# pedrosecchi67/ImmersedBoundary.jl

Hardware: AMD Instinct MI355X
Metric: Mcells*iters/s residual sweep (advection-JST-MUSCL), 2D RAE2822 (higher is better)
Workload: dtype f32

## Files before the change

### immersedboundary.jl_amd/csrc/ibh_common.h

```cpp
#pragma once
#include <hip/hip_runtime.h>
#include <stdint.h>
#include <string>
#include <vector>

#include "../../include/ibhip.h"

#define IBH_MAXD 3

enum : int32_t { SIDE_SAME = 0, SIDE_MIRROR = 1, SIDE_COARSE = 2, SIDE_FINE = 3, SIDE_GENERAL = 4 };

struct BlockDesc2 {
    int32_t base;
    int32_t type[4];
    int32_t nb[4][2];
    int32_t sub[4];
    float h[2];
    float rh[2];
    float q[4];
    float rt[4];
    int32_t dt;
};

struct QuadDesc2 {
    int32_t base;
    uint32_t cls;
    float rh[2];
};
#define IBH_QROW 160
#define IBH_QAUX 40
struct QuadSet2 {
    std::vector<QuadDesc2> qd;
    std::vector<int32_t> qtab;
    std::vector<int32_t> qaux, paux;
    std::vector<int32_t> singles;
    int32_t nq_int = 0, ns_int = 0;
    std::vector<QuadDesc2> pd;
    std::vector<int32_t> ptab;
    std::vector<int32_t> singles2;
};

struct BlockDesc3 {
    int32_t base;
    int32_t fine;
    int32_t type[6];
    int32_t nb[6];
    int32_t sub[6];
    float h[3];
    float rh[3];
    float q[6];
    float rt[6];
};

struct DimData {
    int32_t nf = 0;
    int32_t *owners = nullptr, *neighbors = nullptr;
    int32_t *loff = nullptr, *lidx = nullptr;
    int32_t *roff = nullptr, *ridx = nullptr;
};

struct ibh_part {
    int nd = 0;
    int32_t nc = 0;
    float* spacing = nullptr;
    float* centers = nullptr;
    DimData dim[IBH_MAXD];
    int32_t* side = nullptr;
    int32_t n_image = 0;
    int32_t* image_in_domain = nullptr;
    int bs = 0;
    int32_t nblk = 0;
    int32_t nA1 = 0, nB1 = 0;
    BlockDesc2* blocks2 = nullptr;
    int32_t* htab = nullptr;
    int32_t* etab = nullptr;
    int32_t* dtab = nullptr;
    int32_t n_dt = 0;
    int32_t* img_list = nullptr;
    int32_t n_img = 0, n_img_int = 0, img_all_fz = 0;
    int32_t fuse_all = 0;
    int32_t rows_ok = 0;
    QuadDesc2* qd[2] = {nullptr, nullptr};
    int32_t* qtab[2] = {nullptr, nullptr};
    int32_t* qaux[2] = {nullptr, nullptr};
    int32_t* qsingles[2] = {nullptr, nullptr};
    int32_t nq[2] = {0, 0}, nq_int[2] = {0, 0}, nqs[2] = {0, 0}, nqs_int[2] = {0, 0};
    int32_t npair = 0, nqs2 = 0;
    int32_t* qsingles2 = nullptr;
    int32_t* fz_list = nullptr;
    int32_t* ng_list = nullptr;
    int32_t* nf_list = nullptr;
    int32_t n_fz = 0, n_fz_int = 0, n_ng = 0, n_ng_int = 0, n_nf = 0, n_nf_int = 0;
    BlockDesc3* blocks3 = nullptr;
    int32_t* htab3 = nullptr;
    int32_t* ftab3 = nullptr;
    int32_t *rtab3 = nullptr, *r4tab3 = nullptr;
    int32_t sweep3 = 0;
    BlockDesc3* iblocks3 = nullptr;
    int32_t *ihtab3 = nullptr, *iftab3 = nullptr, *irtab3 = nullptr, *ir4tab3 = nullptr, *idtab3 = nullptr;
    int32_t n_img3 = 0, img_all3 = 0;
    int32_t n_irr = 0;
    int32_t* irr_cells = nullptr;
    int32_t* irr_rec = nullptr;
    int64_t info[24] = {0};
    float* G = nullptr;
    float* march_tmp = nullptr;
    size_t march_tmp_n = 0;
    size_t G_bytes = 0;
};

struct ibh_acc {
    int32_t n_out = 0, n_in = 0;
    int32_t *off = nullptr, *idx = nullptr;
    float* w = nullptr;
    float* packed = nullptr;
};

struct ibh_bc {
    int32_t ng = 0, nid = 0;
    int32_t *ghost = nullptr, *image_domain = nullptr;
    float* eta = nullptr;
    ibh_acc interp;
    std::vector<int32_t> h_ghost, h_off, h_donor;
    std::vector<float> h_eta, h_w;
};

#define IBH_MAX_BC 8
struct ibh_bcset {
    int nbc = 0, nlev = 0;
    int32_t ng = 0;
    int32_t seg[IBH_MAX_BC + 1] = {0};
    bool direct[IBH_MAX_BC] = {false};
    unsigned int* sync = nullptr;
    int32_t *ghost = nullptr, *off = nullptr, *donor = nullptr, *bidx = nullptr;
    float *eta = nullptr, *w = nullptr, *gval = nullptr, *value = nullptr;
    int32_t* mode = nullptr;
};

extern "C" int ibh_shear_rate_of_velocity_cells(const ibh_part* p, const float* vel, int64_t ldv, float* S, float* Gout,
                                                int64_t ldg);
extern "C" int ibh_wray_agarwal_of_cells(const ibh_part* p, const float* R, const float* S, float sigmaR, float C1,
                                         float kappa, float* nut, float* nuR, float* Sout);

extern "C" int ibh_scalar_transport_blocks(const ibh_part* p, const float* R, const float* nuR, float nu, const float* vel,
                                           int64_t ldv, const float* S, float* out, int* done);

extern "C" int ibh_bcset_apply_with_dt(const ibh_bcset* s, float* a, ibh_part* p, const float* C, int64_t ldc, float scale,
                                       float* dt_next, int partials_done);

extern "C" {
extern int ibh_viscous_per_cell;
extern int ibh_ew_scalar_only;
extern int ibh_time_average_nt;
}

extern thread_local std::string ibh_err;
extern thread_local hipStream_t ibh_stream;

int ibh_fail(int code, const char* what, const char* file, int line);

#define IBH_HIP(call)                                                        \
// ... 72 lines not shown
```

### immersedboundary.jl_amd/csrc/ibh_fused.hip

```cpp
#include <algorithm>

#include <string.h>

#include "ibh_common.h"
#include "ibh_flux.h"

using namespace ibhf;

namespace {

struct PartView {
    int32_t nc;
    const float* spacing;
    DimData dim[IBH_MAXD];
    const int32_t* side;
};

struct SideIter {
    int32_t b, e, o, n;
    const int32_t* idx;
    bool direct;
};
__device__ __forceinline__ SideIter side_iter(const PartView& p, int d, int side, int32_t c) {
    const DimData& dd = p.dim[d];
    SideIter it;
    it.idx = side ? dd.ridx : dd.lidx;
    const int32_t t = p.side[(int64_t)(2 * d + side) * p.nc + c];
    it.direct = t >= 0;
    it.o = side ? c : t;
    it.n = side ? t : c;
    if (t >= 0) {
        it.b = 0;
        it.e = 1;
    } else if (t == -2) {
        it.b = it.e = 0;
    } else {
        const int32_t* off = side ? dd.roff : dd.loff;
        it.b = off[c];
        it.e = off[c + 1];
    }
    return it;
}
__device__ __forceinline__ void side_face(const DimData& dd, const SideIter& it, int32_t k, int32_t& o, int32_t& n) {
    if (it.direct) {
        o = it.o;
        n = it.n;
    } else {
        const int32_t f = it.idx[k];
        o = dd.owners[f];
        n = dd.neighbors[f];
    }
}

template <int ND, int NV>
// ... 1125 lines not shown
            F = F * 1.0f;
        }
        Hf[s * 64 + lane] = F;
    }
    blk2::wave_lds_sync();
    const int i = lane & 7, j = lane >> 3;
    const bool e0 = i == 0, e1 = i == 7, e2 = j == 0, e3 = j == 7;
    const float fzl = Hf[4 * 64 + lane], fzh = Hf[5 * 64 + lane];
#pragma unroll
    for (int k = 0; k < 8; ++k) {
        const uint32_t c = base + lane + 64 * k;
        const float *r = tR + k * 64, *t = tT + k * 64, *ax = tAx + k * 64, *ay = tAy + k * 64;
        const float Rc = Rk[k], Tc = Tk[k];
        float fl[3], fr[3];
        const int xl = e0 ? lane : lane - 1, xr = e1 ? lane : lane + 1, yl = e2 ? lane : lane - 8, yr = e3 ? lane : lane + 8;
        const float fxl = tr3_flux(r[xl], Rc, t[xl], Tc, ax[xl], Ak[0][k], h[0], h[0]) * 1.0f;
        const float fxr = tr3_flux(Rc, r[xr], Tc, t[xr], Ak[0][k], ax[xr], h[0], h[0]) * 1.0f;
        const float fyl = tr3_flux(r[yl], Rc, t[yl], Tc, ay[yl], Ak[1][k], h[1], h[1]) * 1.0f;
        const float fyr = tr3_flux(Rc, r[yr], Tc, t[yr], Ak[1][k], ay[yr], h[1], h[1]) * 1.0f;
        fl[0] = e0 ? Hf[0 * 64 + j + 8 * k] : fxl;
        fr[0] = e1 ? Hf[1 * 64 + j + 8 * k] : fxr;
        fl[1] = e2 ? Hf[2 * 64 + i + 8 * k] : fyl;
        fr[1] = e3 ? Hf[3 * 64 + i + 8 * k] : fyr;
        const int kl = k > 0 ? k - 1 : 0, kh = k < 7 ? k + 1 : 7;
        const float fzl_in = tr3_flux(Rk[kl], Rc, Tk[kl], Tc, Ak[2][kl], Ak[2][k], h[2], h[2]) * 1.0f;
        const float fzr_in = tr3_flux(Rc, Rk[kh], Tc, Tk[kh], Ak[2][k], Ak[2][kh], h[2], h[2]) * 1.0f;
        fl[2] = k == 0 ? fzl : fzl_in;
        fr[2] = k == 7 ? fzh : fzr_in;
        float rt = ldg(S, c);
#pragma unroll
        for (int d = 0; d < 3; ++d) rt = rt + (fr[d] - fl[d]) / h[d];
        out[c] = rt;
    }
}


int env_int(const char* name, int dflt) {
    const char* s = getenv(name);
    return s ? atoi(s) : dflt;
}
struct Tuning {
    int wave3d = env_int("IBH_3D_WAVE", 1);
    int sweep_iters = env_int("IBH_SWEEP_ITERS", 0);
    int quad = env_int("IBH_QUAD", 1);
    int rows = env_int("IBH_ROWS", 0);
    int quad_variant = env_int("IBH_QUAD_VARIANT", 0);
    int quad_parts = 3, quad_singles_iters = 1;
    int quad_singles_first = env_int("IBH_SINGLES_FIRST", 0);
    int pairs = env_int("IBH_PAIRS", 1);
    int arith_ids = env_int("IBH_ARITH_IDS", 1);
    int transport_blocks = 1;
    int rows_singles = env_int("IBH_ROWS_SINGLES", -1);
} T;
#define IBH_ROWS_SINGLES_MIN 24000

enum : int {
    QV_STAMPS = 4,
    QV_GATHER_5 = 5, QV_GATHER_69 = 69, QV_GATHER_85 = 85, QV_GATHER_NONE = 100,
    QV_GATHER_SEVEN = 126,
    QV_THREAD_PER_CELL = 512,
    QV_STRIP_W2 = 515, QV_STRIP_W4 = 514, QV_STRIP_W3 = 518,
    QV_COLS_W4 = 519, QV_COLS_W5 = 520,
    QV_EULER_PERSISTENT = 514,
};

constexpr int F_LITERAL = IBH_FORCE_GENERAL | IBH_EXACT;
constexpr int F_TWO_KERNEL = IBH_NO_FUSE | IBH_PASS_A_ONLY | IBH_PASS_B_ONLY;
constexpr int F_PHASES = IBH_PHASE_INTERIOR | IBH_PHASE_BOUNDARY;

bool has_blocks(const ibh_part* p) { return p->bs == 8 && p->nblk > 0 && (p->nd == 2 ? !!p->blocks2 : !!p->blocks3); }
bool tuned2(const ibh_part* p, int flags) { return p->nd == 2 && has_blocks(p) && !(flags & F_LITERAL); }
bool tuned3(const ibh_part* p, int flags) { return p->nd == 3 && has_blocks(p) && !(flags & F_LITERAL); }
bool fused2(const ibh_part* p, int flags) { return tuned2(p, flags) && !(flags & F_TWO_KERNEL); }
bool whole3(const ibh_part* p, int flags) { return tuned3(p, flags) && !(flags & (F_TWO_KERNEL | F_PHASES)); }
bool image3(const ibh_part* p, int flags) { return whole3(p, flags) && (flags & IBH_IMAGE_ONLY) && p->img_all3; }
bool single3(const ibh_part* p, int flags) { return whole3(p, flags) && !(flags & IBH_IMAGE_ONLY) && p->sweep3; }
bool all_blocks3(const ibh_part* p) {
    return p->nd == 3 && has_blocks(p) && p->n_irr == 0 && (int64_t)p->nblk * 512 == p->nc && p->info[6] == 0;
}
bool quads_usable(const ibh_part* p, int k, int flags) { return T.quad && !(flags & IBH_NO_QUAD) && p->nq[k] > 0; }

struct Range { int32_t first, last; int32_t count() const { return last - first; } };
struct Phase {
    bool interior, boundary;
    explicit Phase(int flags) : interior((flags & IBH_PHASE_INTERIOR) != 0), boundary((flags & IBH_PHASE_BOUNDARY) != 0) {}
    bool any() const { return interior || boundary; }
    bool valid() const { return !(interior && boundary); }
    Range of(int32_t n_int, int32_t n_all) const { return {boundary ? n_int : 0, interior ? n_int : n_all}; }
};
#define IBH_PHASES_EXCLUSIVE "IBH_PHASE_INTERIOR and IBH_PHASE_BOUNDARY are exclusive"

PartView view(const ibh_part* p) { return {p->nc, p->spacing, {p->dim[0], p->dim[1], p->dim[2]}, p->side}; }
FlatRec flat_of(const ibh_part* p, const int32_t* cells) {
    return cells && cells == p->irr_cells && p->irr_rec ? FlatRec{p->irr_rec, p->n_irr} : FlatRec{nullptr, 0};
}

int ensure_G(ibh_part* p) {
    if (p->G) return 0;
    hipStreamCaptureStatus st = hipStreamCaptureStatusNone;
    if (ibh_stream && hipStreamIsCapturing(ibh_stream, &st) == hipSuccess && st != hipStreamCaptureStatusNone)
        return ibh_fail(-1, "the gradient workspace is allocated on the first two-kernel sweep of a partition: run one "
                            "sweep before capturing it into a HIP graph", __FILE__, __LINE__);
    const size_t bytes = (size_t)(p->nd * (p->nd + 2) + 1) * (size_t)p->nc * sizeof(float);
    IBH_HIP(hipMalloc((void**)&p->G, bytes));
    p->G_bytes = bytes;
    return 0;
}

struct AdvArgs { const float *u, *C; int64_t ldc; float* ud; };
struct EulerArgs { const float* P; int64_t ldp; float* R; int64_t ldr; const ibh_fluid* fluid; };

struct QuadRange { Range q, s; };
QuadRange quad_range(const ibh_part* p, int k, Phase ph) {
    QuadRange r{ph.of(p->nq_int[k], p->nq[k]), ph.of(p->nqs_int[k], p->nqs[k])};
    if (T.quad_parts == 1) r.s.last = r.s.first;
    if (T.quad_parts == 2) r.q.last = r.q.first;
    return r;
}

struct BlockList { const BlockDesc2* bl; const int32_t *ht, *et, *ls; int32_t count, iters, nwg; };
BlockList block_list(const ibh_part* p, const int32_t* list, Range r, int wpb, int max_iters) {
    const int32_t count = r.count(), iters = T.sweep_iters > 0 ? T.sweep_iters : std::min(max_iters, std::max(1, count / 6000));
    return {list ? p->blocks2 : p->blocks2 + r.first, list ? p->htab : p->htab + (size_t)r.first * 64,
            list ? p->etab : p->etab + (size_t)r.first * 16, list ? list + r.first : nullptr, count, iters,
            (count + wpb * iters - 1) / (wpb * iters)};
}

struct Blocks3 { Range a, b; int32_t nI, gI; bool doA, doB; PartView v; FlatRec flat; };
Blocks3 blocks3_setup(const ibh_part* p, int flags, Phase ph) {
    const Range a = ph.of(p->nA1, p->nblk), b = ph.of(p->nB1, p->nblk);
    const int32_t nI = ph.interior ? 0 : p->n_irr, gI = (nI + 511) / 512;
    return {a, b, nI, gI, !(flags & IBH_PASS_B_ONLY) && (a.count() > 0 || gI), !(flags & IBH_PASS_A_ONLY) && (b.count() > 0 || gI),
            view(p), flat_of(p, p->irr_cells)};
}

struct CellLists { const int32_t *cellsA, *cellsB; int32_t nA, nB; };
CellLists cell_lists(const ibh_part* p, int flags, bool fast, Phase ph) {
    const bool image = (flags & IBH_IMAGE_ONLY) && !fast;
    const int32_t* cellsA = fast ? p->irr_cells : nullptr;
    const int32_t nA = fast ? (ph.interior ? 0 : p->n_irr) : p->nc;
    return {cellsA, image ? p->image_in_domain : cellsA, nA, image ? p->n_image : nA};
}
}

enum AdvPath {
    ADV3_IMAGE_COLS,
    ADV3_SINGLE,
    ADV3_BLOCKS,
    ADV2_IMAGE,
    ADV2_FUSE_ALL,
    ADV2_MIXED,
    ADV_GENERAL_2D,
    ADV_GENERAL_2D_EXACT,
    ADV_GENERAL_3D,
};
static AdvPath advection_path(const ibh_part* p, int flags) {
    if (tuned3(p, flags)) return image3(p, flags) ? ADV3_IMAGE_COLS : single3(p, flags) ? ADV3_SINGLE : ADV3_BLOCKS;
    if (fused2(p, flags)) {
        if ((flags & IBH_IMAGE_ONLY) && p->img_all_fz && !p->fuse_all) return ADV2_IMAGE;
        if (p->fuse_all) return ADV2_FUSE_ALL;
        const bool mixed_pays = p->n_fz >= 12000 || (flags & (IBH_FORCE_MIXED | IBH_SWEEP_ONLY));
        if (p->fz_list && 4 * (int64_t)p->n_fz >= p->nblk && mixed_pays) return ADV2_MIXED;
    }
    return p->nd != 2 ? ADV_GENERAL_3D : (flags & IBH_EXACT) ? ADV_GENERAL_2D_EXACT : ADV_GENERAL_2D;
}

static void adv3_image_cols(const ibh_part* p, const AdvArgs& a) {
    const int32_t nwg = (p->n_img3 + WPB3C - 1) / WPB3C;
    hipLaunchKernelGGL((k_sweep3_cols<3, true>), dim3(nwg), dim3(64 * WPB3C), 0, ibh_stream, a.u, a.C, (uint32_t)a.ldc, a.ud,
                       p->iblocks3, p->ihtab3, p->iftab3, p->irtab3, p->ir4tab3, p->n_img3, nwg, p->idtab3);
}
#define SWEEP3_LAUNCH(K)                                                                                                 \
    hipLaunchKernelGGL(K, dim3(nwg), dim3(64 * WPB3S), 0, ibh_stream, a.u, a.C, (uint32_t)a.ldc, a.ud, p->blocks3, p->htab3, \
                       p->ftab3, p->rtab3, p->r4tab3, p->nblk, nwg)
static void adv3_single(const ibh_part* p, const AdvArgs& a) {
    static_assert(WPB3C == WPB3S, "one grid for both forms");
    const int32_t nwg = (p->nblk + WPB3S - 1) / WPB3S;
    switch (T.quad_variant) {
    case QV_THREAD_PER_CELL:
        hipLaunchKernelGGL(k_sweep3_adv, dim3(p->nblk), dim3(512), 0, ibh_stream, a.u, a.C, (uint32_t)a.ldc, a.ud, p->blocks3,
                           p->htab3, p->ftab3, p->rtab3, p->r4tab3, p->nblk);
        break;
    case QV_STRIP_W2: SWEEP3_LAUNCH(k_sweep3_strip<2>); break;
    case QV_STRIP_W4: SWEEP3_LAUNCH(k_sweep3_strip<4>); break;
    case QV_STRIP_W3: SWEEP3_LAUNCH(k_sweep3_strip<3>); break;
    case QV_COLS_W4: SWEEP3_LAUNCH(k_sweep3_cols<4>); break;
    case QV_COLS_W5: SWEEP3_LAUNCH(k_sweep3_cols<5>); break;
    default: SWEEP3_LAUNCH(k_sweep3_cols<3>);
    }
}
#undef SWEEP3_LAUNCH

static int adv3_blocks(ibh_part* p, const AdvArgs& a, int flags, Phase ph) {
    if (const int rc = ensure_G(p)) return rc;
    const Blocks3 s = blocks3_setup(p, flags, ph);
    const int32_t na = s.a.count(), nb = s.b.count();
    if (s.doA && T.wave3d) {
        const int32_t nwgA = (na + 3) / 4, gIw = (s.nI + 255) / 256;
        hipLaunchKernelGGL(k_passA3_wave, dim3(nwgA + gIw), dim3(256), 0, ibh_stream, s.v, a.u, p->G, p->blocks3 + s.a.first,
                           p->htab3 + (size_t)s.a.first * 384, p->ftab3, na, nwgA, p->irr_cells, s.nI, s.flat,
                           (const int32_t*)nullptr);
    } else if (s.doA)
        hipLaunchKernelGGL(k_passA3_blk, dim3(na + s.gI), dim3(512), 0, ibh_stream, s.v, a.u, p->G, p->blocks3 + s.a.first,
                           p->htab3 + (size_t)s.a.first * 384, p->ftab3, na, p->irr_cells, s.nI, s.flat);
    if (s.doB)
        hipLaunchKernelGGL(k_passB3_adv_blk, dim3(nb + s.gI), dim3(512), 0, ibh_stream, s.v, a.u, a.C, a.ldc, p->G, a.ud,
                           p->blocks3 + s.b.first, p->htab3 + (size_t)s.b.first * 384, p->ftab3, nb, p->irr_cells, s.nI,
                           s.flat, (const int32_t*)nullptr);
    return 0;
}

static void adv2_block_list(const ibh_part* p, const AdvArgs& a, const int32_t* list, Range r) {
    if (r.count() <= 0) return;
    const BlockList L = block_list(p, list, r, WPB, 6);
    hipLaunchKernelGGL(p->n_dt > 0 ? k_sweep_adv<true> : k_sweep_adv<false>, dim3(L.nwg), dim3(64 * WPB), 0, ibh_stream, a.u,
                       a.C, (uint32_t)a.ldc, a.ud, L.bl, L.ht, L.et, p->dtab, L.count, L.nwg, L.iters, L.ls);
}

static void adv2_quads(const ibh_part* p, const AdvArgs& a, int k, Phase ph) {
    const Range q = quad_range(p, k, ph).q;
    Range s = quad_range(p, k, ph).s;
    const int32_t npair = (k == 0 && T.pairs && p->npair > 0 && !ph.boundary && q.first == 0 && q.last == p->nq[k] &&
                           T.quad_parts == 3) ? p->npair : 0;
    const int32_t* slist = p->qsingles[k];
    if (npair) {
        slist = p->qsingles2;
        s = {0, p->nqs2};
    } else if (k == 0 && p->npair > 0 && ph.boundary) {
        s.last = s.first;
    }
    const bool rows_able = k == 0 && p->rows_ok && p->n_dt == 0 && T.quad_variant == 0 && s.count() > 0;
    const bool rows_inside = rows_able && T.rows_singles == 2;
    const bool rows_second = rows_able && !rows_inside &&
                             (T.rows_singles < 0 ? s.count() >= IBH_ROWS_SINGLES_MIN : T.rows_singles > 0);
    const Range rs = s;
    if (rows_second) s.last = s.first;
    const int32_t siters = T.quad_singles_iters > 0 ? T.quad_singles_iters : 1;
    const int32_t nwgq = (q.count() + npair + WPB - 1) / WPB,
                  nwgs = rows_inside ? (s.count() + WPB * 8 - 1) / (WPB * 8) : (s.count() + WPB * siters - 1) / (WPB * siters);
    auto kq = k_sweep_quad<false, false>;
    if (rows_inside) kq = k_sweep_quad<false, false, 127, false, true>;
    else if (p->n_dt > 0) kq = k_sweep_quad<true, false>;
    else if (T.quad_variant == QV_STAMPS) kq = k_sweep_quad<false, true>;
    else if (T.quad_variant == QV_GATHER_SEVEN) kq = k_sweep_quad<false, false, 126>;
    else if (T.quad_variant == QV_GATHER_85) kq = k_sweep_quad<false, false, 85>;
    else if (T.quad_variant == QV_GATHER_69) kq = k_sweep_quad<false, false, 69>;
    else if (T.quad_variant == QV_GATHER_5) kq = k_sweep_quad<false, false, 5>;
    else if (T.quad_variant == QV_GATHER_NONE) kq = k_sweep_quad<false, false, 0>;
    if (nwgq + nwgs > 0)
        hipLaunchKernelGGL(kq, dim3(nwgq + nwgs), dim3(64 * WPB), 0, ibh_stream, a.u, a.C, (uint32_t)a.ldc, a.ud,
                           p->qd[k] + q.first, p->qtab[k] + (size_t)q.first * IBH_QROW, q.count(), nwgq, p->blocks2, p->htab,
                           p->etab, p->dtab, slist + s.first, s.count(), nwgs, T.quad_singles_first, siters,
                           (const float*)nullptr, npair,
                           T.arith_ids ? p->qaux[k] + (size_t)q.first * IBH_QAUX : (const int32_t*)nullptr);
    if (rows_second) {
        const int32_t nw = (rs.count() + 7) / 8, nwgr = (nw + WPBR - 1) / WPBR;
        hipLaunchKernelGGL(k_sweep_rows, dim3(nwgr), dim3(64 * WPBR), 0, ibh_stream, a.u, a.C, (uint32_t)a.ldc, a.ud,
                           p->blocks2, p->etab, 0, rs.count(), nwgr, slist + rs.first);
    }
}

static void adv2_single(const ibh_part* p, const AdvArgs& a, int flags, Phase ph, int k) {
    const Range b = k ? ph.of(p->n_img_int, p->n_img) : ph.of(p->nB1, p->nblk);
    if (k == 0 && p->rows_ok && T.rows && !(flags & IBH_NO_QUAD) && T.quad_variant == 0) {
        const int32_t nw = (b.count() + 7) / 8, nwg = (nw + WPBR - 1) / WPBR;
        if (nwg > 0)
            hipLaunchKernelGGL(k_sweep_rows, dim3(nwg), dim3(64 * WPBR), 0, ibh_stream, a.u, a.C, (uint32_t)a.ldc, a.ud,
                               p->blocks2, p->etab, b.first, b.count(), nwg, (const int32_t*)nullptr);
    } else if (quads_usable(p, k, flags)) adv2_quads(p, a, k, ph);
    else adv2_block_list(p, a, k ? p->img_list : nullptr, b);
}

static int adv2_mixed(ibh_part* p, const AdvArgs& a, int flags, Phase ph) {
    const bool defer = p->n_nf_int == 0;
    const Range g = ph.of(defer ? 0 : p->n_ng_int, p->n_ng), r = ph.of(p->n_nf_int, p->n_nf);
    const int32_t nI = ph.interior ? 0 : p->n_irr, gI = (nI + 64 * WPB - 1) / (64 * WPB);
    if (const int rc = ensure_G(p)) return rc;
    const int32_t nwgA = (g.count() + WPB - 1) / WPB, nwgB = (r.count() + WPB - 1) / WPB;
    if (!(flags & IBH_SWEEP_ONLY)) {
        const PartView v = view(p);
        if (nwgA + gI)
            hipLaunchKernelGGL((k_passA<2, 1, false>), dim3(nwgA + gI), dim3(64 * WPB), 0, ibh_stream, v, a.u, (int64_t)p->nc,
                               p->G, p->blocks2, p->htab, g.count(), nwgA, p->irr_cells, nI, flat_of(p, p->irr_cells),
                               p->ng_list + g.first);
        if (nwgB + gI)
            hipLaunchKernelGGL((k_passB_adv<2, false>), dim3(nwgB + gI), dim3(64 * WPB), 0, ibh_stream, v, a.u, a.C, a.ldc,
                               p->G, a.ud, p->blocks2, p->htab, r.count(), nwgB, p->irr_cells, nI,
                               flat_of(p, p->irr_cells), p->nf_list + r.first);
    }
    adv2_block_list(p, a, p->fz_list, ph.of(p->n_fz_int, p->n_fz));
    return 0;
}

static int adv_general(ibh_part* p, const AdvArgs& a, int flags, Phase ph, AdvPath path) {
    if (const int rc = ensure_G(p)) return rc;
    const bool fast = p->nd == 2 && has_blocks(p) && !(flags & IBH_FORCE_GENERAL);
    IBH_REQUIRE(!ph.any() || fast, "overlap phases need the block path (2-D, block_size 8, domain given)");
    const Range ra = ph.of(p->nA1, p->nblk), rb = ph.of(p->nB1, p->nblk);
    const int32_t nwgA = fast ? (ra.count() + WPB - 1) / WPB : 0, nwgB = fast ? (rb.count() + WPB - 1) / WPB : 0;
    const CellLists c = cell_lists(p, flags, fast, ph);
    const PartView v = view(p);
    const dim3 blk(64 * WPB), gA(nwgA + (c.nA + 64 * WPB - 1) / (64 * WPB)), gB(nwgB + (c.nB + 64 * WPB - 1) / (64 * WPB));
    const bool doA = gA.x && !(flags & IBH_PASS_B_ONLY), doB = gB.x && !(flags & IBH_PASS_A_ONLY);
    const BlockDesc2 *blkA = p->blocks2 ? p->blocks2 + ra.first : nullptr, *blkB = p->blocks2 ? p->blocks2 + rb.first : nullptr;
    const int32_t* htA = p->htab ? p->htab + (size_t)ra.first * 64 : nullptr;
    const int32_t* htB = p->htab ? p->htab + (size_t)rb.first * 64 : nullptr;
    const bool d3 = path == ADV_GENERAL_3D, exact = path == ADV_GENERAL_2D_EXACT;
    auto kA = d3 ? k_passA<3, 1, true> : exact ? k_passA<2, 1, true> : k_passA<2, 1, false>;
    auto kB = d3 ? k_passB_adv<3, true> : exact ? k_passB_adv<2, true> : k_passB_adv<2, false>;
    if (doA)
        hipLaunchKernelGGL(kA, gA, blk, 0, ibh_stream, v, a.u, (int64_t)p->nc, p->G, blkA, htA, ra.count(), nwgA, c.cellsA, c.nA,
                           flat_of(p, c.cellsA), (const int32_t*)nullptr);
    if (doB)
        hipLaunchKernelGGL(kB, gB, blk, 0, ibh_stream, v, a.u, a.C, a.ldc, p->G, a.ud, blkB, htB, rb.count(), nwgB, c.cellsB,
                           c.nB, flat_of(p, c.cellsB), (const int32_t*)nullptr);
    return 0;
}

enum EulerPath {
    EUL2_SINGLE,
    EUL3_IMAGE_COLS,
    EUL3_SINGLE,
    EUL2_FAST,
    EUL2_FACE_LIST,
// ... 58 lines not shown
    } else if (s.doA)
        hipLaunchKernelGGL(k_passA3e_blk, dim3(p->nblk + s.gI), dim3(512), 0, ibh_stream, s.v, e.P, e.ldp, p->G, p->blocks3,
                           p->htab3, p->ftab3, p->nblk, p->irr_cells, s.nI, s.flat);
    if (s.doB) {
        hipLaunchKernelGGL(k_passB3e_blk, dim3(p->nblk), dim3(512), 0, ibh_stream, (uint32_t)p->nc, e.P, (uint32_t)e.ldp,
                           p->G, e.R, (uint32_t)e.ldr, e.fluid->R, e.fluid->gamma, p->blocks3, p->htab3, p->ftab3, p->nblk);
        if (s.nI)
            hipLaunchKernelGGL((k_passB_euler<3>), dim3((s.nI + 64 * WPB - 1) / (64 * WPB)), dim3(64 * WPB), 0, ibh_stream,
                               s.v, e.P, e.ldp, p->G, e.R, e.ldr, e.fluid->R, e.fluid->gamma, p->irr_cells, s.nI);
    }
    return 0;
}

static int euler_general(ibh_part* p, const EulerArgs& e, int flags, EulerPath path) {
    if (const int rc = ensure_G(p)) return rc;
    const PartView v = view(p);
    const bool fast = path == EUL2_FAST;
    const int32_t nwg_fast = fast ? (p->nblk + WPB - 1) / WPB : 0;
    const CellLists c = cell_lists(p, flags, fast, Phase(0));
    const dim3 blk(64 * WPB), gA(nwg_fast + (c.nA + 64 * WPB - 1) / (64 * WPB)), gB((c.nB + 64 * WPB - 1) / (64 * WPB));
    const bool doA = gA.x && !(flags & IBH_PASS_B_ONLY), doB = !(flags & IBH_PASS_A_ONLY);
    auto kA = fast ? k_passA<2, 4, false> : path == EUL2_FACE_LIST ? k_passA<2, 4, true> : k_passA<3, 5, true>;
    if (doA)
        hipLaunchKernelGGL(kA, gA, blk, 0, ibh_stream, v, e.P, e.ldp, p->G, p->blocks2, p->htab, p->nblk, nwg_fast, c.cellsA,
                           c.nA, flat_of(p, c.cellsA), (const int32_t*)nullptr);
    if (doB && nwg_fast)
        hipLaunchKernelGGL(k_passB_euler_blk, dim3(nwg_fast), blk, 0, ibh_stream, (uint32_t)p->nc, e.P, (uint32_t)e.ldp, p->G,
                           e.R, (uint32_t)e.ldr, e.fluid->R, e.fluid->gamma, p->blocks2, p->htab, p->nblk, nwg_fast);
    if (doB && gB.x)
        hipLaunchKernelGGL(path == EUL3_FACE_LIST ? k_passB_euler<3> : k_passB_euler<2>, gB, blk, 0, ibh_stream, v, e.P, e.ldp,
                           p->G, e.R, e.ldr, e.fluid->R, e.fluid->gamma, c.cellsB, c.nB);
    return 0;
}

extern "C" {

int ibh_debug_buffer(void* buf) {
    unsigned long long* b = (unsigned long long*)buf;
    IBH_HIP(hipMemcpyToSymbol(HIP_SYMBOL(ibh_dbg_buf), &b, sizeof(b)));
    return 0;
}

int ibh_set_tuning(const char* key, int value) {
    static const struct { const char* key; int* value; } keys[] = {
        {"viscous_per_cell", &ibh_viscous_per_cell}, {"ew_scalar", &ibh_ew_scalar_only},
        {"time_average_nt", &ibh_time_average_nt},
        {"quad_variant", &T.quad_variant}, {"quad_parts", &T.quad_parts}, {"quad_singles_first", &T.quad_singles_first},
        {"quad_singles_iters", &T.quad_singles_iters}, {"rows", &T.rows}, {"rows_singles", &T.rows_singles},
        {"transport_blocks", &T.transport_blocks}, {"pairs", &T.pairs}, {"arith_ids", &T.arith_ids}};
    IBH_REQUIRE(key, "ibh_set_tuning: null key");
    for (const auto& k : keys)
        if (!strcmp(key, k.key)) {
            *k.value = value;
            return 0;
        }
    return ibh_fail(-1, "ibh_set_tuning: unknown key", __FILE__, __LINE__);
}

int ibh_residual_advection(ibh_part* p, const float* u, const float* C, int64_t ldc, float* ud, int flags) {
    IBH_REQUIRE(p && u && C && ud, "ibh_residual_advection: null argument");
    if (p->nc == 0) return 0;
    const Phase ph(flags);
    IBH_REQUIRE(ph.valid(), IBH_PHASES_EXCLUSIVE);
    const AdvArgs a{u, C, ldc, ud};
    const AdvPath path = advection_path(p, flags);
    int rc = 0;
    switch (path) {
    case ADV3_IMAGE_COLS: adv3_image_cols(p, a); break;
    case ADV3_SINGLE: adv3_single(p, a); break;
    case ADV3_BLOCKS: rc = adv3_blocks(p, a, flags, ph); break;
    case ADV2_IMAGE: adv2_single(p, a, flags, ph, 1); break;
    case ADV2_FUSE_ALL: adv2_single(p, a, flags, ph, 0); break;
    case ADV2_MIXED: rc = adv2_mixed(p, a, flags, ph); break;
    default: rc = adv_general(p, a, flags, ph, path);
    }
    if (!rc) IBH_LAUNCH_CHECK();
    return rc;
}

int ibh_residual_advection_n(ibh_part* p, const float* u, const float* C, int64_t ldc, float* ud, int flags, int n) {
    int rc = 0;
    for (int i = 0; i < n && !rc; ++i) rc = ibh_residual_advection(p, u, C, ldc, ud, flags);
    return rc;
}

int ibh_residual_euler_hll(ibh_part* p, const float* P, int64_t ldp, float* R, int64_t ldr, const ibh_fluid* fluid,
                           int flags) {
    IBH_REQUIRE(p && P && R && fluid, "ibh_residual_euler_hll: null argument");
    if (p->nc == 0) return 0;
    const Phase ph(flags);
    const EulerArgs e{P, ldp, R, ldr, fluid};
    const EulerPath path = euler_path(p, flags);
    if (path == EUL2_SINGLE) IBH_REQUIRE(ph.valid(), IBH_PHASES_EXCLUSIVE);
    else
        IBH_REQUIRE(!ph.any(), "ibh_residual_euler_hll: overlap phases need a partition whose (image) blocks are all "
                               "eligible for the single-kernel sweep; run the sweep unphased after the exchange");
    int rc = 0;
    switch (path) {
    case EUL2_SINGLE: euler2_single(p, e, flags, ph); break;
    case EUL3_IMAGE_COLS: euler3_image_cols(p, e); break;
    case EUL3_SINGLE: euler3_single(p, e); break;
    case EUL3_BLOCKS: rc = euler3_blocks(p, e, flags); break;
    default: rc = euler_general(p, e, flags, path);
    }
    if (!rc) IBH_LAUNCH_CHECK();
    return rc;
}

int ibh_step_advection(ibh_part* p, const float* u, float* u_out, const float* C, int64_t ldc, const float* dt_dev,
                       const ibh_bcset* bcs) {
    IBH_REQUIRE(p && u && u_out && C && dt_dev && u != u_out, "ibh_step_advection: null or aliased argument");
    if (p->nc == 0) return 0;
    int rc = 0;
    if (fused2(p, 0) && p->fuse_all && quads_usable(p, 0, 0) && p->n_dt == 0) {
        const int32_t npair = T.pairs ? p->npair : 0;
        const int32_t nq = p->nq[0], ns = npair ? p->nqs2 : p->nqs[0];
        const int32_t nwgq = (nq + npair + WPB - 1) / WPB, nwgs = (ns + WPB - 1) / WPB;
        hipLaunchKernelGGL((k_sweep_quad<false, false, 127, true>), dim3(nwgq + nwgs), dim3(64 * WPB), 0, ibh_stream, u, C,
                           (uint32_t)ldc, u_out, p->qd[0], p->qtab[0], nq, nwgq, p->blocks2, p->htab, p->etab, p->dtab,
                           npair ? p->qsingles2 : p->qsingles[0], ns, nwgs, T.quad_singles_first, 1, dt_dev, npair,
                           T.arith_ids ? p->qaux[0] : (const int32_t*)nullptr);
        IBH_LAUNCH_CHECK();
    } else {
        if ((rc = ibh_residual_advection(p, u, C, ldc, u_out, 0))) return rc;
        if ((rc = ibh_update_dev(p->nc, dt_dev, u, u_out, u_out))) return rc;
    }
    if (bcs) rc = ibh_bcset_apply(bcs, u_out);
    return rc;
}

int ibh_step_advection_dt(ibh_part* p, const float* u, float* u_out, const float* C, int64_t ldc, const float* dt_dev,
                          const ibh_bcset* bcs, float scale, float* dt_next) {
    IBH_REQUIRE(dt_next, "ibh_step_advection_dt: null dt_next");
    int rc = ibh_step_advection(p, u, u_out, C, ldc, dt_dev, nullptr);
    if (rc) return rc;
    if (bcs && bcs->ng > 0) return ibh_bcset_apply_with_dt(bcs, u_out, p, C, ldc, scale, dt_next, 0);
    return ibh_timestep_advection(p, C, ldc, scale, dt_next);
}

int ibh_step_advection_xgmi(ibh_part* p, float* u, const float* C, int64_t ldc, float* ud, const int32_t* send_all,
                            int n_send_peers, const int32_t* send_seg, float* const* dst0, float* const* dst1,
                            uint32_t* const* send_flags, const int32_t* recv_all, const float* src0, const float* src1,
                            int n_recv_peers, const int32_t* recv_seg, const uint32_t* const* recv_flags,
                            uint32_t* state, uint32_t max_spins, unsigned long long* fstate) {
    IBH_REQUIRE(p && u && C && ud && state && fstate, "ibh_step_advection_xgmi: null argument");
    IBH_REQUIRE(fused2(p, 0) && p->img_all_fz && !p->fuse_all && quads_usable(p, 1, 0),
                "ibh_step_advection_xgmi: needs a 2-D partition with skirt fragments whose image blocks are all eligible "
                "for the quad sweep");
    IBH_REQUIRE(n_send_peers >= 0 && n_send_peers <= IBH_MAX_PEERS && n_recv_peers >= 0 && n_recv_peers <= IBH_MAX_PEERS &&
                    n_send_peers + n_recv_peers > 0,
                "ibh_step_advection_xgmi: 1 to 16 peers");
    XchgArgs A;
    memset(&A, 0, sizeof(A));
    A.ns = n_send_peers;
    A.nr = n_recv_peers;
    if (n_send_peers) {
        IBH_REQUIRE(send_all && send_seg && dst0 && dst1 && send_flags, "ibh_step_advection_xgmi: null send argument");
        for (int q = 0; q < n_send_peers; ++q) {
            A.dst[0][q] = dst0[q];
            A.dst[1][q] = dst1[q];
            A.sflag[q] = send_flags[q];
            A.sseg[q] = send_seg[q];
        }
        A.sseg[n_send_peers] = send_seg[n_send_peers];
    }
    if (n_recv_peers) {
        IBH_REQUIRE(recv_all && src0 && src1 && recv_seg && recv_flags, "ibh_step_advection_xgmi: null receive argument");
        for (int q = 0; q < n_recv_peers; ++q) {
            A.rflag[q] = recv_flags[q];
            A.rseg[q] = recv_seg[q];
        }
        A.rseg[n_recv_peers] = recv_seg[n_recv_peers];
    }
    const int32_t big = std::max(A.ns ? A.sseg[A.ns] : 0, A.nr ? A.rseg[A.nr] : 0);
// ... 105 lines not shown
```

Baseline: 120,000.

## Cache prebuilt kernel-argument records and launch sweeps via hipModuleLaunchKernel

Adds a per-partition cache of launch records (function handle, grid and packed kernel-argument buffer) for the common 2D advection residual and step sweeps, keyed by flags and invalidated by a tuning epoch. Repeated calls only patch the leading u/C/ldc/ud (and dt) fields and launch through hipModuleLaunchKernel with an extra-args buffer. This skips the per-call path selection and argument marshalling on the host. In exchange it relies on static_asserts tying the struct layout to the kernel signatures, and adds cache-invalidation complexity.

After: 121,300, median of 4. Within noise of the previous version (+1.1%).

```diff
diff --git a/immersedboundary.jl_amd/csrc/ibh_common.h b/immersedboundary.jl_amd/csrc/ibh_common.h
--- a/immersedboundary.jl_amd/csrc/ibh_common.h
+++ b/immersedboundary.jl_amd/csrc/ibh_common.h
@@ -57,6 +57,18 @@
     int32_t *owners = nullptr, *neighbors = nullptr;
     int32_t *loff = nullptr, *lidx = nullptr;
     int32_t *roff = nullptr, *ridx = nullptr;
+};
+
+#define IBH_REC_ARG_BYTES 144
+#define IBH_REC_ENTRIES 2
+#define IBH_REC_SLOTS 4
+struct ibh_launch_rec {
+    int epoch = 0, flags = 0;
+    int path = -1;
+    hipFunction_t fn = nullptr;
+    uint32_t grid = 0, wg = 0;
+    uint32_t bytes = 0;
+    alignas(16) unsigned char args[IBH_REC_ARG_BYTES] = {0};
 };
 
 struct ibh_part {
@@ -107,6 +119,8 @@
     float* march_tmp = nullptr;
     size_t march_tmp_n = 0;
     size_t G_bytes = 0;
+    ibh_launch_rec rec[IBH_REC_ENTRIES][IBH_REC_SLOTS];
+    int rec_next[IBH_REC_ENTRIES] = {0};
 };
 
 struct ibh_acc {
diff --git a/immersedboundary.jl_amd/csrc/ibh_fused.hip b/immersedboundary.jl_amd/csrc/ibh_fused.hip
--- a/immersedboundary.jl_amd/csrc/ibh_fused.hip
+++ b/immersedboundary.jl_amd/csrc/ibh_fused.hip
@@ -1,5 +1,7 @@
 #include <algorithm>
-
+#include <type_traits>
+
+#include <stddef.h>
 #include <string.h>
 
 #include "ibh_common.h"
@@ -1231,6 +1233,7 @@
     int transport_blocks = 1;
     int rows_singles = env_int("IBH_ROWS_SINGLES", -1);
 } T;
+int tuning_epoch = 1;
 #define IBH_ROWS_SINGLES_MIN 24000
 
 enum : int {
@@ -1321,6 +1324,52 @@
     return {cellsA, image ? p->image_in_domain : cellsA, nA, image ? p->n_image : nA};
 }
 }
+
+struct QuadArgs {
+    const float *u, *C; uint32_t ldc; float* ud;
+    const QuadDesc2* qd; const int32_t* qtab; int32_t nq, nwgq; const BlockDesc2* blocks;
+    const int32_t *htab, *etab, *dtab, *singles; int32_t ns, nwgs, singles_first, siters;
+    const float* dtp; int32_t npair; const int32_t* qaux;
+};
+struct BlockArgs {
+    const float *u, *C; uint32_t ldc; float* ud;
+    const BlockDesc2* bl; const int32_t *ht, *et, *dtab; int32_t count, nwg, iters; const int32_t* ls;
+};
+struct SweepHead { const float *u, *C; uint32_t ldc; float* ud; };
+#define ARG(S, m) decltype(S::m)
+using QuadKernel = void (*)(ARG(QuadArgs, u), ARG(QuadArgs, C), ARG(QuadArgs, ldc), ARG(QuadArgs, ud), ARG(QuadArgs, qd),
+                            ARG(QuadArgs, qtab), ARG(QuadArgs, nq), ARG(QuadArgs, nwgq), ARG(QuadArgs, blocks),
+                            ARG(QuadArgs, htab), ARG(QuadArgs, etab), ARG(QuadArgs, dtab), ARG(QuadArgs, singles),
+                            ARG(QuadArgs, ns), ARG(QuadArgs, nwgs), ARG(QuadArgs, singles_first), ARG(QuadArgs, siters),
+                            ARG(QuadArgs, dtp), ARG(QuadArgs, npair), ARG(QuadArgs, qaux));
+using BlockKernel = void (*)(ARG(BlockArgs, u), ARG(BlockArgs, C), ARG(BlockArgs, ldc), ARG(BlockArgs, ud), ARG(BlockArgs, bl),
+                             ARG(BlockArgs, ht), ARG(BlockArgs, et), ARG(BlockArgs, dtab), ARG(BlockArgs, count),
+                             ARG(BlockArgs, nwg), ARG(BlockArgs, iters), ARG(BlockArgs, ls));
+#undef ARG
+template <class... A>
+constexpr size_t kernarg_bytes(void (*)(A...)) {
+    size_t off = 0;
+    ((off = (off + alignof(A) - 1) / alignof(A) * alignof(A) + sizeof(A)), ...);
+    return off;
+}
+static_assert(std::is_same<QuadKernel, decltype(&k_sweep_quad<false, false>)>::value &&
+                  std::is_same<QuadKernel, decltype(&k_sweep_quad<true, false>)>::value &&
+                  std::is_same<QuadKernel, decltype(&k_sweep_quad<false, false, 127, true>)>::value,
+              "QuadArgs lists the parameters of k_sweep_quad, in order");
+static_assert(std::is_same<BlockKernel, decltype(&k_sweep_adv<false>)>::value &&
+                  std::is_same<BlockKernel, decltype(&k_sweep_adv<true>)>::value,
+              "BlockArgs lists the parameters of k_sweep_adv, in order");
+static_assert(std::is_standard_layout<QuadArgs>::value && sizeof(QuadArgs) == kernarg_bytes(QuadKernel()) &&
+                  sizeof(QuadArgs) == 136 && offsetof(QuadArgs, dtp) == 112 && offsetof(QuadArgs, qaux) == 128,
+              "QuadArgs is laid out as the kernel-argument segment of k_sweep_quad");
+static_assert(std::is_standard_layout<BlockArgs>::value && sizeof(BlockArgs) == kernarg_bytes(BlockKernel()) &&
+                  sizeof(BlockArgs) == 88 && offsetof(BlockArgs, ls) == 80,
+              "BlockArgs is laid out as the kernel-argument segment of k_sweep_adv");
+#define HEAD_AT(S) (offsetof(S, u) == offsetof(SweepHead, u) && offsetof(S, C) == offsetof(SweepHead, C) && \
+                    offsetof(S, ldc) == offsetof(SweepHead, ldc) && offsetof(S, ud) == offsetof(SweepHead, ud))
+static_assert(HEAD_AT(QuadArgs) && HEAD_AT(BlockArgs) && offsetof(SweepHead, ud) == 24, "the patched fields lead both blocks");
+#undef HEAD_AT
+static_assert(sizeof(QuadArgs) <= IBH_REC_ARG_BYTES && sizeof(BlockArgs) <= IBH_REC_ARG_BYTES, "a record holds either block");
 
 enum AdvPath {
     ADV3_IMAGE_COLS,
@@ -1389,14 +1438,23 @@
     return 0;
 }
 
+struct BlockPlan { BlockKernel kb; int32_t nwg; BlockArgs a; };
+static BlockPlan block_plan(const ibh_part* p, const int32_t* list, Range r) {
+    if (r.count() <= 0) return {nullptr, 0, {}};
+    const BlockList L = block_list(p, list, r, WPB, 6);
+    return {p->n_dt > 0 ? k_sweep_adv<true> : k_sweep_adv<false>, L.nwg,
+            {nullptr, nullptr, 0, nullptr, L.bl, L.ht, L.et, p->dtab, L.count, L.nwg, L.iters, L.ls}};
+}
 static void adv2_block_list(const ibh_part* p, const AdvArgs& a, const int32_t* list, Range r) {
-    if (r.count() <= 0) return;
-    const BlockList L = block_list(p, list, r, WPB, 6);
-    hipLaunchKernelGGL(p->n_dt > 0 ? k_sweep_adv<true> : k_sweep_adv<false>, dim3(L.nwg), dim3(64 * WPB), 0, ibh_stream, a.u,
-                       a.C, (uint32_t)a.ldc, a.ud, L.bl, L.ht, L.et, p->dtab, L.count, L.nwg, L.iters, L.ls);
-}
-
-static void adv2_quads(const ibh_part* p, const AdvArgs& a, int k, Phase ph) {
+    const BlockPlan P = block_plan(p, list, r);
+    if (P.nwg <= 0) return;
+    const BlockArgs& b = P.a;
+    hipLaunchKernelGGL(P.kb, dim3(P.nwg), dim3(64 * WPB), 0, ibh_stream, a.u, a.C, (uint32_t)a.ldc, a.ud, b.bl, b.ht, b.et,
+                       b.dtab, b.count, b.nwg, b.iters, b.ls);
+}
+
+struct QuadPlan { QuadKernel kq; int32_t nwg; QuadArgs a; bool rows_second; Range rs; const int32_t* slist; };
+static QuadPlan quad_plan(const ibh_part* p, int k, Phase ph) {
     const Range q = quad_range(p, k, ph).q;
     Range s = quad_range(p, k, ph).s;
     const int32_t npair = (k == 0 && T.pairs && p->npair > 0 && !ph.boundary && q.first == 0 && q.last == p->nq[k] &&
@@ -1417,7 +1475,7 @@
     const int32_t siters = T.quad_singles_iters > 0 ? T.quad_singles_iters : 1;
     const int32_t nwgq = (q.count() + npair + WPB - 1) / WPB,
                   nwgs = rows_inside ? (s.count() + WPB * 8 - 1) / (WPB * 8) : (s.count() + WPB * siters - 1) / (WPB * siters);
-    auto kq = k_sweep_quad<false, false>;
+    QuadKernel kq = k_sweep_quad<false, false>;
     if (rows_inside) kq = k_sweep_quad<false, false, 127, false, true>;
     else if (p->n_dt > 0) kq = k_sweep_quad<true, false>;
     else if (T.quad_variant == QV_STAMPS) kq = k_sweep_quad<false, true>;
@@ -1426,16 +1484,23 @@
     else if (T.quad_variant == QV_GATHER_69) kq = k_sweep_quad<false, false, 69>;
     else if (T.quad_variant == QV_GATHER_5) kq = k_sweep_quad<false, false, 5>;
     else if (T.quad_variant == QV_GATHER_NONE) kq = k_sweep_quad<false, false, 0>;
-    if (nwgq + nwgs > 0)
-        hipLaunchKernelGGL(kq, dim3(nwgq + nwgs), dim3(64 * WPB), 0, ibh_stream, a.u, a.C, (uint32_t)a.ldc, a.ud,
-                           p->qd[k] + q.first, p->qtab[k] + (size_t)q.first * IBH_QROW, q.count(), nwgq, p->blocks2, p->htab,
-                           p->etab, p->dtab, slist + s.first, s.count(), nwgs, T.quad_singles_first, siters,
-                           (const float*)nullptr, npair,
-                           T.arith_ids ? p->qaux[k] + (size_t)q.first * IBH_QAUX : (const int32_t*)nullptr);
-    if (rows_second) {
-        const int32_t nw = (rs.count() + 7) / 8, nwgr = (nw + WPBR - 1) / WPBR;
+    return {kq, nwgq + nwgs,
+            {nullptr, nullptr, 0, nullptr, p->qd[k] + q.first, p->qtab[k] + (size_t)q.first * IBH_QROW, q.count(), nwgq,
+             p->blocks2, p->htab, p->etab, p->dtab, slist + s.first, s.count(), nwgs, T.quad_singles_first, siters, nullptr,
+             npair, T.arith_ids ? p->qaux[k] + (size_t)q.first * IBH_QAUX : (const int32_t*)nullptr},
+            rows_second, rs, slist};
+}
+static void adv2_quads(const ibh_part* p, const AdvArgs& a, int k, Phase ph) {
+    const QuadPlan P = quad_plan(p, k, ph);
+    const QuadArgs& q = P.a;
+    if (P.nwg > 0)
+        hipLaunchKernelGGL(P.kq, dim3(P.nwg), dim3(64 * WPB), 0, ibh_stream, a.u, a.C, (uint32_t)a.ldc, a.ud, q.qd, q.qtab, q.nq,
+                           q.nwgq, q.blocks, q.htab, q.etab, q.dtab, q.singles, q.ns, q.nwgs, q.singles_first, q.siters,
+                           q.dtp, q.npair, q.qaux);
+    if (P.rows_second) {
+        const int32_t nw = (P.rs.count() + 7) / 8, nwgr = (nw + WPBR - 1) / WPBR;
         hipLaunchKernelGGL(k_sweep_rows, dim3(nwgr), dim3(64 * WPBR), 0, ibh_stream, a.u, a.C, (uint32_t)a.ldc, a.ud,
-                           p->blocks2, p->etab, 0, rs.count(), nwgr, slist + rs.first);
+                           p->blocks2, p->etab, 0, P.rs.count(), nwgr, P.slist + P.rs.first);
     }
 }
 
@@ -1449,6 +1514,80 @@
     } else if (quads_usable(p, k, flags)) adv2_quads(p, a, k, ph);
     else adv2_block_list(p, a, k ? p->img_list : nullptr, b);
 }
+
+enum RecEntry { REC_ADVECTION = 0, REC_STEP = 1 };
+static_assert(REC_STEP < IBH_REC_ENTRIES, "one record set per entry");
+
+template <class Args, class Kernel>
+static int rec_fill(ibh_launch_rec& r, Kernel k, int32_t nwg, const Args& a) {
+    if (nwg <= 0) return 0;
+    hipFunction_t fn = nullptr;
+    IBH_HIP(hipGetFuncBySymbol(&fn, (const void*)k));
+    memcpy(r.args, &a, sizeof(Args));
+    r.bytes = sizeof(Args);
+    r.grid = (uint32_t)nwg;
+    r.wg = 64 * WPB;
+    r.fn = fn;
+    return 0;
+}
+
+static int step_record(const ibh_part* p, ibh_launch_rec& r);
+static int rec_build(const ibh_part* p, RecEntry entry, int flags, ibh_launch_rec& r) {
+    r = ibh_launch_rec();
+    r.flags = flags;
+    if (entry == REC_STEP) return step_record(p, r);
+    const Phase ph(flags);
+    const AdvPath path = advection_path(p, flags);
+    r.path = path;
+    if (ph.any() || (path != ADV2_IMAGE && path != ADV2_FUSE_ALL)) return 0;
+    const int k = path == ADV2_IMAGE ? 1 : 0;
+    if (k == 0 && p->rows_ok && T.rows && !(flags & IBH_NO_QUAD) && T.quad_variant == 0) return 0;
+    if (quads_usable(p, k, flags)) {
+        const QuadPlan P = quad_plan(p, k, ph);
+        const bool dflt = P.kq == QuadKernel(k_sweep_quad<false, false>) || P.kq == QuadKernel(k_sweep_quad<true, false>);
+        if (!dflt || P.rows_second || T.quad_variant != 0 || T.quad_parts != 3) return 0;
+        return rec_fill(r, P.kq, P.nwg, P.a);
+    }
+    const BlockPlan B = block_plan(p, k ? p->img_list : nullptr, k ? ph.of(p->n_img_int, p->n_img) : ph.of(p->nB1, p->nblk));
+    return rec_fill(r, B.kb, B.nwg, B.a);
+}
+
+static const ibh_launch_rec* rec_get(ibh_part* p, RecEntry entry, int flags, int* rc) {
+    ibh_launch_rec* set = p->rec[entry];
+    for (int i = 0; i < IBH_REC_SLOTS; ++i)
+        if (set[i].epoch == tuning_epoch && set[i].flags == flags) return set + i;
+    ibh_launch_rec& r = set[p->rec_next[entry]];
+    p->rec_next[entry] = (p->rec_next[entry] + 1) % IBH_REC_SLOTS;
+    if ((*rc = rec_build(p, entry, flags, r))) {
+        r.epoch = 0;
+        return nullptr;
+    }
+    r.epoch = tuning_epoch;
+    return &r;
+}
+
+struct RecCall {
+    alignas(16) unsigned char kb[IBH_REC_ARG_BYTES];
+    size_t bytes;
+    void* extra[5];
+    const ibh_launch_rec& r;
+    RecCall(const ibh_launch_rec& rec, const float* u, const float* C, int64_t ldc, float* ud, const float* dtp) : r(rec) {
+        memcpy(kb, r.args, r.bytes);
+        SweepHead* h = (SweepHead*)kb;
+        h->u = u;
+        h->C = C;
+        h->ldc = (uint32_t)ldc;
+        h->ud = ud;
+        if (dtp) ((QuadArgs*)kb)->dtp = dtp;
+        bytes = r.bytes;
+        extra[0] = HIP_LAUNCH_PARAM_BUFFER_POINTER;
+        extra[1] = kb;
+        extra[2] = HIP_LAUNCH_PARAM_BUFFER_SIZE;
+        extra[3] = &bytes;
+        extra[4] = HIP_LAUNCH_PARAM_END;
+    }
+    hipError_t launch() { return hipModuleLaunchKernel(r.fn, r.grid, 1, 1, r.wg, 1, 1, 0, ibh_stream, nullptr, extra); }
+};
 
 static int adv2_mixed(ibh_part* p, const AdvArgs& a, int flags, Phase ph) {
     const bool defer = p->n_nf_int == 0;
@@ -1613,17 +1752,15 @@
     for (const auto& k : keys)
         if (!strcmp(key, k.key)) {
             *k.value = value;
+            ++tuning_epoch;
             return 0;
         }
     return ibh_fail(-1, "ibh_set_tuning: unknown key", __FILE__, __LINE__);
 }
 
-int ibh_residual_advection(ibh_part* p, const float* u, const float* C, int64_t ldc, float* ud, int flags) {
-    IBH_REQUIRE(p && u && C && ud, "ibh_residual_advection: null argument");
-    if (p->nc == 0) return 0;
+static int advection_by_launcher(ibh_part* p, const AdvArgs& a, int flags) {
     const Phase ph(flags);
     IBH_REQUIRE(ph.valid(), IBH_PHASES_EXCLUSIVE);
-    const AdvArgs a{u, C, ldc, ud};
     const AdvPath path = advection_path(p, flags);
     int rc = 0;
     switch (path) {
@@ -1640,9 +1777,25 @@
 }
 
 int ibh_residual_advection_n(ibh_part* p, const float* u, const float* C, int64_t ldc, float* ud, int flags, int n) {
+    if (n <= 0) return 0;
+    IBH_REQUIRE(p && u && C && ud, "ibh_residual_advection: null argument");
+    if (p->nc == 0) return 0;
     int rc = 0;
-    for (int i = 0; i < n && !rc; ++i) rc = ibh_residual_advection(p, u, C, ldc, ud, flags);
+    const ibh_launch_rec* r = rec_get(p, REC_ADVECTION, flags, &rc);
+    if (!r) return rc;
+    if (r->fn) {
+        RecCall call(*r, u, C, ldc, ud, nullptr);
+        for (int i = 0; i < n; ++i) IBH_HIP(call.launch());
+        IBH_LAUNCH_CHECK();
+        return 0;
+    }
+    const AdvArgs a{u, C, ldc, ud};
+    for (int i = 0; i < n && !rc; ++i) rc = advection_by_launcher(p, a, flags);
     return rc;
+}
+
+int ibh_residual_advection(ibh_part* p, const float* u, const float* C, int64_t ldc, float* ud, int flags) {
+    return ibh_residual_advection_n(p, u, C, ldc, ud, flags, 1);
 }
 
 int ibh_residual_euler_hll(ibh_part* p, const float* P, int64_t ldp, float* R, int64_t ldr, const ibh_fluid* fluid,
@@ -1668,19 +1821,27 @@
     return rc;
 }
 
+static int step_record(const ibh_part* p, ibh_launch_rec& r) {
+    if (!(fused2(p, 0) && p->fuse_all && quads_usable(p, 0, 0) && p->n_dt == 0)) return 0;
+    const int32_t npair = T.pairs ? p->npair : 0;
+    const int32_t nq = p->nq[0], ns = npair ? p->nqs2 : p->nqs[0];
+    const int32_t nwgq = (nq + npair + WPB - 1) / WPB, nwgs = (ns + WPB - 1) / WPB;
+    r.path = ADV2_FUSE_ALL;
+    return rec_fill(r, QuadKernel(k_sweep_quad<false, false, 127, true>), nwgq + nwgs,
+                    QuadArgs{nullptr, nullptr, 0, nullptr, p->qd[0], p->qtab[0], nq, nwgq, p->blocks2, p->htab, p->etab,
+                             p->dtab, npair ? p->qsingles2 : p->qsingles[0], ns, nwgs, T.quad_singles_first, 1, nullptr,
+                             npair, T.arith_ids ? p->qaux[0] : (const int32_t*)nullptr});
+}
+
 int ibh_step_advection(ibh_part* p, const float* u, float* u_out, const float* C, int64_t ldc, const float* dt_dev,
                        const ibh_bcset* bcs) {
     IBH_REQUIRE(p && u && u_out && C && dt_dev && u != u_out, "ibh_step_advection: null or aliased argument");
     if (p->nc == 0) return 0;
     int rc = 0;
-    if (fused2(p, 0) && p->fuse_all && quads_usable(p, 0, 0) && p->n_dt == 0) {
-        const int32_t npair = T.pairs ? p->npair : 0;
-        const int32_t nq = p->nq[0], ns = npair ? p->nqs2 : p->nqs[0];
-        const int32_t nwgq = (nq + npair + WPB - 1) / WPB, nwgs = (ns + WPB - 1) / WPB;
-        hipLaunchKernelGGL((k_sweep_quad<false, false, 127, true>), dim3(nwgq + nwgs), dim3(64 * WPB), 0, ibh_stream, u, C,
-                           (uint32_t)ldc, u_out, p->qd[0], p->qtab[0], nq, nwgq, p->blocks2, p->htab, p->etab, p->dtab,
-                           npair ? p->qsingles2 : p->qsingles[0], ns, nwgs, T.quad_singles_first, 1, dt_dev, npair,
-                           T.arith_ids ? p->qaux[0] : (const int32_t*)nullptr);
+    const ibh_launch_rec* r = rec_get(p, REC_STEP, 0, &rc);
+    if (!r) return rc;
+    if (r->fn) {
+        IBH_HIP(RecCall(*r, u, C, ldc, u_out, dt_dev).launch());
         IBH_LAUNCH_CHECK();
     } else {
         if ((rc = ibh_residual_advection(p, u, C, ldc, u_out, 0))) return rc;
```
